# navganti/SIVO

Hardware: AMD Instinct MI355X
Metric: frames/sec, SIVO per-frame path (ORB+SegNet T=12+entropy) 352x1024 (higher is better)
Workload: dtype f32 (f16x3)

## Files before the change

### include/sivo_hip.h

```cpp
#ifndef SIVO_HIP_H
#define SIVO_HIP_H

#include <stddef.h>
#include <stdint.h>

#ifdef __cplusplus
extern "C" {
#endif

#define SIVO_OK 0
#define SIVO_ERR_INVALID_ARGUMENT 1
#define SIVO_ERR_RUNTIME 2
#define SIVO_ERR_UNSUPPORTED 3
#define SIVO_ERR_IMAGE_TOO_SMALL 4
#define SIVO_ERR_CAPACITY 5

const char *sivo_last_error(void);
int sivo_version(void);
int sivo_device_count(void);

typedef struct sivo_segnet *sivo_segnet_t;

int sivo_segnet_create(const char *prototxt_text, size_t prototxt_len, int t_override,
                       const float *weights, size_t n_weights, int device, sivo_segnet_t *out);
typedef struct SivoSegnetOptions {
    uint32_t struct_size;
    int32_t lanes;
    int32_t gemm;
    int32_t no_direct_f16x3;
    int32_t no_packed_activations;
    int32_t conv7_fp32;
    int32_t wino4_workspace_mb;
    int32_t debug_sync;
} SivoSegnetOptions;
int sivo_segnet_create_opts(const char *prototxt_text, size_t prototxt_len, int t_override, const float *weights, size_t n_weights,
                            int device, const SivoSegnetOptions *opts, sivo_segnet_t *out);
int sivo_caffemodel_weights(const char *prototxt_text, size_t prototxt_len, const void *model_bytes,
                            size_t model_len, float *out, size_t capacity, size_t *n_weights);
int sivo_segnet_create_from_files(const char *model_file, const char *weights_file, int t_override,
                                  int device, sivo_segnet_t *out);
int sivo_segnet_create_from_files_opts(const char *model_file, const char *weights_file, int t_override, int device,
                                       const SivoSegnetOptions *opts, sivo_segnet_t *out);
int sivo_segnet_create_multi(const char *prototxt_text, size_t prototxt_len, int t_override, const float *weights,
                             size_t n_weights, const int *device_ids, int ndev, sivo_segnet_t *out);
int sivo_segnet_create_multi_from_files(const char *model_file, const char *weights_file, int t_override,
                                        const int *device_ids, int ndev, sivo_segnet_t *out);
int sivo_segnet_create_multi_opts(const char *prototxt_text, size_t prototxt_len, int t_override, const float *weights, size_t n_weights,
                                  const int *device_ids, int ndev, const SivoSegnetOptions *opts, sivo_segnet_t *out);
int sivo_segnet_create_multi_from_files_opts(const char *model_file, const char *weights_file, int t_override, const int *device_ids,
                                             int ndev, const SivoSegnetOptions *opts, sivo_segnet_t *out);
int sivo_segnet_num_devices(sivo_segnet_t h, int *ndev);
int sivo_segnet_destroy(sivo_segnet_t h);
int sivo_segnet_shape(sivo_segnet_t h, int32_t *T, int32_t *C, int32_t *H, int32_t *W, int32_t *classes);
int sivo_segnet_num_params(const char *prototxt_text, size_t prototxt_len, size_t *n_params);

int sivo_segnet_forward_dev(sivo_segnet_t h, const uint8_t *d_bgr, int n_samples, int sample0,
// ... 22 lines not shown
int sivo_segnet_segment_logits_dev(sivo_segnet_t h, const uint8_t *d_bgr, uint64_t seed, uint8_t *d_classes,
                                   double *d_confidence, double *d_entropy, float *d_logits, void *stream);

int sivo_mc_segment_dev(const float *d_logits, int T, int classes, int64_t hw, uint8_t *d_classes,
                        double *d_confidence, double *d_entropy, void *stream);

int sivo_segnet_blob(sivo_segnet_t h, const char *name, float *host_out, size_t capacity, int32_t shape[4]);

int sivo_segnet_flops(sivo_segnet_t h, double *shared, double *per_sample);

typedef struct {
    char layer[64];
    char kernel[96];
    int32_t samples;
    int32_t launches;
    double flops_per_sample;
    double bytes_per_sample;
    double ms_total;
    int32_t kernel_launches;
    int32_t pad_;
} SivoOpProfile;
int sivo_segnet_profile(sivo_segnet_t h, int enable);
int sivo_segnet_profile_read(sivo_segnet_t h, SivoOpProfile *out, int capacity, int *n_out);

typedef struct SivoH3Layer {
    char layer[48];
    float vmax, vscale, uscale;
} SivoH3Layer;
int sivo_segnet_gemm_status(sivo_segnet_t h, int *mode, int *overflow_frames, SivoH3Layer *per_layer, int capacity, int *n_layers);
typedef struct SivoGuardLayer {
    char layer[48];
    char kernel[24];
    float rel_err, rel_rms, ref_max, first_rel_err;
    int32_t level;
} SivoGuardLayer;
int sivo_segnet_guard_report(sivo_segnet_t h, SivoGuardLayer *rows, int capacity, int *n_rows, float *budget, float *predicted,
                             float *logit_max, double *guard_ms, int *builds);
int sivo_segnet_take_overflow(sivo_segnet_t h, int *overflowed);

typedef struct {
    float x, y, size, angle, response;
    int32_t octave, class_id;
} SivoKeyPoint;

typedef struct sivo_orb *sivo_orb_t;

// ... 322 lines not shown
```

### sivo_amd/_lib.py

```python
import ctypes as C
import os
import threading

_HERE = os.path.dirname(os.path.abspath(__file__))
LIB_PATH = os.path.join(_HERE, "libsivo_hip.so")

OK = 0
ERR_INVALID_ARGUMENT = 1
ERR_RUNTIME = 2
ERR_UNSUPPORTED = 3
ERR_IMAGE_TOO_SMALL = 4
ERR_CAPACITY = 5


class SivoError(RuntimeError):
    def __init__(self, code, msg):
        super().__init__(f"libsivo_hip error {code}: {msg}")
        self.code = code


class SivoInvalidArgument(SivoError, ValueError):
    """SIVO_ERR_INVALID_ARGUMENT: where the reference throws std::invalid_argument."""


class KeyPoint(C.Structure):
    _fields_ = [("x", C.c_float), ("y", C.c_float), ("size", C.c_float), ("angle", C.c_float),
                ("response", C.c_float), ("octave", C.c_int32), ("class_id", C.c_int32)]


class OpProfile(C.Structure):
    _fields_ = [("layer", C.c_char * 64), ("kernel", C.c_char * 96), ("samples", C.c_int32), ("launches", C.c_int32),
                ("flops_per_sample", C.c_double), ("bytes_per_sample", C.c_double), ("ms_total", C.c_double),
                ("kernel_launches", C.c_int32), ("pad_", C.c_int32)]


class SegnetOptions(C.Structure):
    _fields_ = [("struct_size", C.c_uint32), ("lanes", C.c_int32), ("gemm", C.c_int32), ("no_direct_f16x3", C.c_int32),
                ("no_packed_activations", C.c_int32), ("conv7_fp32", C.c_int32), ("wino4_workspace_mb", C.c_int32), ("debug_sync", C.c_int32)]


class SearchQuery(C.Structure):
    _fields_ = [("u", C.c_float), ("v", C.c_float), ("radius", C.c_float), ("lvl_lo", C.c_int32), ("lvl_hi", C.c_int32),
                ("ur", C.c_float), ("gate", C.c_float), ("angle", C.c_float), ("flags", C.c_int32)]


class SearchRule(C.Structure):
    _fields_ = [("th_dist", C.c_int32), ("accept_lt", C.c_int32), ("ratio_mode", C.c_int32), ("nn_ratio", C.c_float),
                ("gate_mode", C.c_int32), ("check_orientation", C.c_int32), ("dynamic", C.c_int32), ("tie_last", C.c_int32),
                ("F12", C.c_float * 9), ("ex", C.c_float), ("ey", C.c_float)]


class Edge(C.Structure):
    _fields_ = [("pose", C.c_int32), ("point", C.c_int32), ("stereo", C.c_int32), ("pad_", C.c_int32),
                ("obs", C.c_double * 3), ("inv_sigma2", C.c_double)]


class Sim3Match(C.Structure):
    _fields_ = [("obs1", C.c_double * 2), ("inv_sigma2_1", C.c_double), ("obs2", C.c_double * 2), ("inv_sigma2_2", C.c_double),
                ("x1c", C.c_double * 3), ("x2c", C.c_double * 3)]


# ... 60 lines not shown
    "sivo_segnet_create_from_files_opts": [C.c_char_p, C.c_char_p, _i, _i, _vp, C.POINTER(_vp)],
    "sivo_segnet_create_multi_opts": [C.c_char_p, _sz, _i, _vp, _sz, _pi32, _i, _vp, C.POINTER(_vp)],
    "sivo_segnet_create_multi_from_files_opts": [C.c_char_p, C.c_char_p, _i, _pi32, _i, _vp, C.POINTER(_vp)],
    "sivo_caffemodel_weights": [C.c_char_p, _sz, _vp, _sz, _vp, _sz, C.POINTER(_sz)],
    "sivo_segnet_create_from_files": [C.c_char_p, C.c_char_p, _i, _i, C.POINTER(_vp)],
    "sivo_segnet_create_multi": [C.c_char_p, _sz, _i, _vp, _sz, _pi32, _i, C.POINTER(_vp)],
    "sivo_segnet_create_multi_from_files": [C.c_char_p, C.c_char_p, _i, _pi32, _i, C.POINTER(_vp)],
    "sivo_segnet_num_devices": [_vp, _pi32],
    "sivo_segnet_destroy": [_vp],
    "sivo_segnet_shape": [_vp, _pi32, _pi32, _pi32, _pi32, _pi32],
    "sivo_segnet_num_params": [C.c_char_p, _sz, C.POINTER(_sz)],
    "sivo_segnet_forward_dev": [_vp, _vp, _i, _i, _u64, _vp, _vp, _vp, _vp],
    "sivo_mc_finalize_dev": [_vp, _i, _i64, _i, _vp, _vp, _vp, _vp],
    "sivo_mc_reduce_dev": [_vp, _i, _i, _i64, _vp, _vp, _i, _vp],
    "sivo_mc_variance_dev": [_vp, _i, _i, _i64, _vp, _vp, _vp],
    "sivo_segnet_segment": [_vp, _vp, _i, _i, _u64, _vp, _vp, _vp],
    "sivo_segnet_segment_dev": [_vp, _vp, _u64, _vp, _vp, _vp, _vp],
    "sivo_segnet_segment_logits_dev": [_vp, _vp, _u64, _vp, _vp, _vp, _vp, _vp],
    "sivo_mc_segment_dev": [_vp, _i, _i, _i64, _vp, _vp, _vp, _vp],
    "sivo_segnet_blob": [_vp, C.c_char_p, _vp, _sz, _pi32],
    "sivo_segnet_flops": [_vp, C.POINTER(_d), C.POINTER(_d)],
    "sivo_segnet_profile": [_vp, _i],
    "sivo_segnet_profile_read": [_vp, _vp, _i, _pi32],
    "sivo_segnet_gemm_status": [_vp, _pi32, _pi32, _vp, _i, _pi32],
    "sivo_segnet_prefix_bands": [_vp, _i, _vp, _vp, _vp],
    "sivo_segnet_prefix_band_dev": [_vp, _vp, _i, _i, _vp, _vp],
    "sivo_segnet_forward_banded_dev": [_vp, _vp, _i, _i, _i, C.c_uint64, _vp, _vp, _vp],
    "sivo_segnet_guard_report": [_vp, _vp, _i, _pi32, _vp, _vp, _vp, _vp, _pi32],
    "sivo_segnet_take_overflow": [_vp, _pi32],
    "sivo_orb_create": [_i, _f, _i, _i, _i, _i, C.POINTER(_vp)],
    "sivo_orb_destroy": [_vp],
    "sivo_orb_set_gaussian": [_vp, _i],
    "sivo_orb_set_launch_mode": [_vp, _i],
    "sivo_orb_tables": [_vp, _vp, _vp, _vp, _vp, _vp],
    "sivo_orb_extract": [_vp, _vp, _i, _i, _i, _vp, _vp, _i, _pi32],
    "sivo_orb_extract_dev": [_vp, _vp, _i, _i, _i, _vp, _vp, _i, _pi32, _vp],
    "sivo_orb_extract_pair_dev": [_vp, _vp, _vp, _vp, _i, _i, _i, _i, _vp, _vp, _i, _pi32, _vp, _vp, _i, _pi32, _vp],
    "sivo_orb_profile": [_vp, _i],
    "sivo_orb_profile_read": [_vp, C.POINTER(_d), _pi32, C.POINTER(_d)],
    "sivo_orb_level": [_vp, _i, _vp, _sz, _pi32, _pi32],
    "sivo_orb_candidates": [_vp, _i, _vp, _i, _pi32],
    "sivo_orb_distribute": [_vp, _i, _i, _i, _i, _i, _i, _vp, _i, _pi32],
    "sivo_hamming_matrix_dev": [_vp, _i, _vp, _i, _vp, _vp],
    "sivo_hamming_matrix": [_vp, _i, _vp, _i, _vp],
    "sivo_hamming_argmin2_dev": [_vp, _i, _vp, _vp, _vp, _vp, _vp, _vp, _vp, _vp],
    "sivo_hamming_argmin2": [_vp, _i, _vp, _i, _vp, _vp, _vp, _vp, _vp, _vp],
# ... 141 lines not shown
```

### sivo_amd/api/bayesian_segnet/bayesian_segnet.hpp

```cpp
#ifndef BAYESIAN_SEGNET_BAYESIAN_SEGNET_HPP
#define BAYESIAN_SEGNET_BAYESIAN_SEGNET_HPP

#ifdef SIVO_HAVE_EIGEN
#include <Eigen/Eigen>
#else
#include "../compat/eigen_min.hpp"
#endif
#ifdef SIVO_HAVE_OPENCV
#include <opencv2/core/core.hpp>
#else
#include "../compat/cv_min.hpp"
#endif

#include <cstdint>
#include <string>
#include <vector>

#include "../../../include/sivo_hip.h"

struct sivo_segnet;

namespace SIVO {

#ifdef SIVO_HAVE_EIGEN
// ... 1 lines not shown
using MatXu = Eigen::Matrix<uint8_t, Eigen::Dynamic, Eigen::Dynamic, Eigen::RowMajor>;
#else
using MatXd = sivo_compat::RowMatrix<double>;
using MatXu = sivo_compat::RowMatrix<uint8_t>;
#endif

double computeEntropy(const double probability);

enum Classes {
    ROAD, SIDEWALK, BUILDING, WALL, POLE, TRAFFIC_LIGHT, TRAFFIC_SIGN, VEGETATION, TERRAIN, SKY, PERSON, CAR,
    COMMERCIAL_VEHICLE, BIKE, VOID = 255
};

struct BayesianSegNetParams {
    BayesianSegNetParams(const std::string model_filepath, const std::string weights_filepath)
        : model_file(model_filepath), weights_file(weights_filepath) {}
    bool use_gpu = true;
    std::string model_file;
    std::string weights_file;
    int monte_carlo_samples = 0;
    uint64_t seed = 0;
    int device = 0;
    std::vector<int> devices;
    SivoSegnetOptions options = {sizeof(SivoSegnetOptions), 0, 0, 0, 0, 0, 0, 0};
};

class BayesianSegNet {
 public:
    explicit BayesianSegNet(const BayesianSegNetParams &params);
    ~BayesianSegNet();
    BayesianSegNet(const BayesianSegNet &) = delete;
    BayesianSegNet &operator=(const BayesianSegNet &) = delete;

    void segmentImage(const cv::Mat &image, MatXu &classes, MatXd &confidence, MatXd &entropy);
    cv::Mat generateConfidenceImage(const MatXd &confidence);
    cv::Mat generateVarianceImage(MatXd &variance);
    cv::Mat generateEntropyImage(MatXd &entropy);
    cv::Mat generateSegmentedImage(const MatXu &classes, const cv::Mat &test_image);
    cv::Size getInputGeometry() { return this->input_geometry; }

 private:
    void checkConfig();
    void generateSegmentationColours();
    cv::Mat resizeImage(const cv::Mat &image);

    sivo_segnet *handle = nullptr;
    cv::Size input_geometry;
// ... 8 lines not shown
```

### sivo_amd/csrc/conv_wino4_h3.hip

```cpp
#include <hip/hip_runtime.h>
#include <stdint.h>

#include <cmath>
#include <cstdlib>
#include <cstring>
#include <vector>

#include "common.hpp"
#include "lds_dma.hpp"
#include "segnet_kernels.hpp"

namespace sivo {

typedef _Float16 half8 __attribute__((ext_vector_type(8)));
typedef float f32x16 __attribute__((ext_vector_type(16)));
typedef uint32_t u32x4 __attribute__((ext_vector_type(4)));
typedef int i32x4 __attribute__((ext_vector_type(4)));

constexpr int H3_KC = 32;

struct H3Args {
    const uint32_t *V;
    const unsigned char *U;
    float *M;
// ... 569 lines not shown
    for (int xi = 0; xi < 36; ++xi)
        for (int cb = 0; cb < ncb; ++cb)
            for (int s = 0; s < nst; ++s) {
                uint16_t *img = out.data() + ((size_t)(xi * ncb + cb) * nst + s) * 2048;
                for (int o = 0; o < 4; ++o)
                    for (int r = 0; r < 32; ++r)
                        for (int el = 0; el < 8; ++el) {
                            const float x = U[((size_t)xi * cin + s * H3_KC + 8 * o + el) * Kp + cb * 32 + r];
                            const uint32_t p = wino4_h3_pack_value(x, scale);
                            const size_t at = (size_t)(o * 32 + r) * 8 + el;
                            img[at] = (uint16_t)(p & 0xffffu);
                            img[1024 + at] = (uint16_t)(p >> 16);
                        }
            }
    return scale;
}

struct H3Tile { int bm, bn; };
static H3Tile h3_tile(int64_t P, int Kp) {
    if (Kp % 256) return {256, 128};
    const int64_t items_big = 36 * ((P + 255) / 256) * (Kp / 256);
    return {items_big >= 3 * 256 ? 256 : 128, 256};
}

void launch_wino4_gemm_h3(const uint32_t *V, const void *U, float *M, int C, int Kp, int P, int Pp, hipStream_t s) {
    static const bool lds_all = !(SIVO_DIAG_ENV("SIVO_H3_LDS_ALL") && std::atoi(SIVO_DIAG_ENV("SIVO_H3_LDS_ALL")) == 0);
    static const int force_tile = SIVO_DIAG_ENV("SIVO_H3_TILE") ? std::atoi(SIVO_DIAG_ENV("SIVO_H3_TILE")) : -1;
    static int attr_set[64] = {0};
    if (FirstUse once(attr_set); once) {
        for (const void *f : {(const void *)wino4_gemm_h3_kernel<256, 256>, (const void *)wino4_gemm_h3_kernel<128, 256>, (const void *)wino4_gemm_h3_kernel<256, 128>})
            SIVO_HIP(hipFuncSetAttribute(f, hipFuncAttributeMaxDynamicSharedMemorySize, 160 * 1024));
    }
    static const int n_cu = [] { hipDeviceProp_t pr; int d = 0; (void)hipGetDevice(&d); return hipGetDeviceProperties(&pr, d) == hipSuccess ? pr.multiProcessorCount : 256; }();
    const dim3 grid((unsigned)((n_cu / 8) * 8 > 0 ? (n_cu / 8) * 8 : 8));
    H3Args a{};
    a.V = V; a.U = static_cast<const unsigned char *>(U); a.M = M; a.C = C; a.Kp = Kp; a.P = P; a.Pp = Pp;
    H3Tile t = h3_tile(P, Kp);
    if (t.bn == 256 && (force_tile == 0 || force_tile == 1)) t.bm = force_tile == 0 ? 256 : 128;
    a.ptiles = (int)((P + t.bm - 1) / t.bm); a.ktiles = Kp / t.bn;
    const size_t lds = lds_all ? (size_t)160 * 1024 : (size_t)(2 * t.bm + 3 * t.bn) * 128;
#ifdef SIVO_DIAG
    if (const char *ab = SIVO_DIAG_ENV("SIVO_H3_ABL")) {
        a.ptiles = (P + 255) / 256; a.ktiles = Kp / 256;
#define H3_ABL_CASE(n)                                                                                                              \
    case n:                                                                                                                         \
        SIVO_HIP(hipFuncSetAttribute(reinterpret_cast<const void *>(wino4_gemm_h3_kernel<256, 256, n>), hipFuncAttributeMaxDynamicSharedMemorySize, 160 * 1024)); \
// ... 47 lines not shown
```

### sivo_amd/csrc/segnet.cpp

```cpp
#include "segnet_impl.hpp"

namespace sivo {

void harvest(sivo_segnet &S) {
    if (!S.pending) return;
    for (Op &op : S.ops) {
        if (!op.timed_mask) continue;
        int n = 0;
        for (int l = 0; l < Op::PROF_LANES; ++l) {
            if (!(op.timed_mask & (1u << l))) continue;
            float ms = 0.f;
            if (!op.w4_gemm_only_last) {
                SIVO_HIP(hipEventSynchronize(op.ev1[l]));
                SIVO_HIP(hipEventElapsedTime(&ms, op.ev0[l], op.ev1[l]));
                op.ms_total += ms;
            }
            for (int g = 0; g < op.w4_groups_last[l]; ++g)
                for (int k = op.w4_gemm_only_last ? 1 : 0; k < (op.w4_gemm_only_last ? 2 : 3); ++k) {
                    SIVO_HIP(hipEventSynchronize(op.w4_ev[l][4 * g + k + 1]));
                    SIVO_HIP(hipEventElapsedTime(&ms, op.w4_ev[l][4 * g + k], op.w4_ev[l][4 * g + k + 1]));
                    op.w4_ms[k] += ms;
                }
            op.w4_launches += op.w4_groups_last[l];
            op.w4_groups_last[l] = 0;
            op.kernel_launches += 1;
            n += op.lane_n[l];
        }
        op.last_n = n;
        op.launches += 1;
        op.timed_mask = 0;
    }
    S.pending = false;
// ... 166 lines not shown
        if (debug_sync) SIVO_HIP(hipDeviceSynchronize());
    }
}

void forward(sivo_segnet &S, const uint8_t *d_bgr, int n, int sample0, uint64_t seed, float *d_prob_sum,
             float *d_logits, float *d_prob, hipStream_t st, const McTargets *mc, const BandInput *pre) {
    const int64_t hw = (int64_t)S.H * S.W;
    S.last_seed = seed; S.last_sample0 = sample0;
    if (S.profile) harvest(S);
    h3_absorb(S);
    struct Pause {
        sivo_segnet &S; bool was;
        explicit Pause(sivo_segnet &s) : S(s), was(s.h3_on) { if (S.h3_pause) S.h3_on = false; S.h3_pause = false; }
        ~Pause() { S.h3_on = was; }
    } pause(S);
    const Blob &lg = S.blobs[S.logits_blob];
    if (lg.shared) throw std::runtime_error("the network has no test-time dropout: nothing to sample");
    if (!pre) launch_preprocess(d_bgr, (float *)S.blobs[S.input_blob].d, hw, st);
    const bool fuse = S.cls_op >= 0 && !d_prob && !d_logits && (mc || d_prob_sum || S.d_sum64);
    const size_t last = fuse ? (size_t)S.cls_op : S.ops.size();
    S.cls_pk_now = fuse && S.ops[S.cls_op].c3 && S.ops[S.cls_op].pk_in && S.ops[S.cls_op].d3_vscale > 0.f && S.pk_on && S.h3_on && !S.calibrating;
    size_t fork = 0;
    while (fork < last && (S.ops[fork].skip || S.blobs[S.ops[fork].out].shared)) ++fork;
    int lanes = S.d_wino4_ws ? S.ws_lanes : 2;
    if (S.profile && !S.profile_keep_lanes) lanes = 1;
    while (lanes > 1 && n < 2 * lanes) --lanes;
    while (lanes > 1 && fork < last && !S.ops[fork].skip && S.ops[fork].out2 >= 0 && S.blobs[S.ops[fork].out2].shared &&
           !S.blobs[S.ops[fork].out].shared)
        ++fork;
    if (pre) bands_unpack(S, *pre, n, sample0, seed, st, &fork);
    else run_ops(S, 0, fork, 0, n, sample0, seed, st, 0);
    if (lanes == 1) {
        run_ops(S, fork, last, 0, n, sample0, seed, st, 0);
    } else {
        if (!S.lane_fork) SIVO_HIP(hipEventCreateWithFlags(&S.lane_fork, hipEventDisableTiming));
        SIVO_HIP(hipEventRecord(S.lane_fork, st));
        int n0 = 0;
        for (int l = 0; l < lanes; ++l) {
            const int nl = n / lanes + (l < n % lanes ? 1 : 0);
            hipStream_t ls = st;
            if (l > 0) {
                if (!S.lane_stream[l]) {
                    SIVO_HIP(hipStreamCreateWithFlags(&S.lane_stream[l], hipStreamNonBlocking));
                    SIVO_HIP(hipEventCreateWithFlags(&S.lane_join[l], hipEventDisableTiming));
                }
                ls = S.lane_stream[l];
                SIVO_HIP(hipStreamWaitEvent(ls, S.lane_fork, 0));
            }
            run_ops(S, fork, last, n0, nl, sample0, seed, ls, l);
            if (l > 0) SIVO_HIP(hipEventRecord(S.lane_join[l], ls));
            n0 += nl;
        }
        for (int l = 1; l < lanes; ++l) SIVO_HIP(hipStreamWaitEvent(st, S.lane_join[l], 0));
    }
    if (fuse) {
        Op &op = S.ops[S.cls_op];
        const Blob &bi = S.blobs[op.in];
        ClsMcArgs a{};
        a.in = (const float *)bi.d; a.in_sample_stride = bi.chw();
        a.wt = op.d_w_mc; a.ep_scale = op.d_scale; a.ep_shift = op.d_shift;
        a.T = n; a.Cin = op.cin; a.H = bi.H; a.W = bi.W; a.C = op.cout; a.relu = op.relu;
        a.logits = mc ? mc->logits : nullptr;
// ... 471 lines not shown
                    p.ms_total = op.w4_ms[k];
                    p.launches = op.launches;
                    p.kernel_launches = op.w4_launches;
                    (void)groups;
                }
                continue;
            }
            SivoOpProfile &p = out[r++];
            std::memset(&p, 0, sizeof p);
            std::snprintf(p.layer, sizeof p.layer, "%s", op.name.c_str());
            const bool d3_on = op.d3 && h->h3_on && op.d3_vscale > 0.f && op.drop_site < 0 && op.pool_op < 0;
            std::snprintf(p.kernel, sizeof p.kernel, "%s", op.mc_fused_last ? (op.cls_h3_last ? "conv_cls_h3_kernel" : "conv_wino_cls_mc_kernel") : d3_on ? "conv3_h3_kernel" : (op.c7h3 && !(h->h3_on && op.d3_vscale > 0.f)) ? "conv7_x6_kernel" : op.kernel.c_str());
            p.samples = op.last_n;
            p.flops_per_sample = op.flops;
            p.bytes_per_sample = op.bytes;
            p.ms_total = op.ms_total;
            p.launches = op.launches;
            p.kernel_launches = op.kernel_launches;
        }
        return SIVO_OK;
    });
}

extern "C" int sivo_segnet_take_overflow(sivo_segnet_t h, int *overflowed) {
    return guarded([&] {
        if (!h || !overflowed) throw std::invalid_argument("null argument");
        if (h->multi) throw std::invalid_argument("a multi-device handle has synchronous entry points only: they recompute such a frame themselves");
        const bool now = h3_tripped(*h);
        *overflowed = (now || h->h3_unreported) ? 1 : 0;
        h->h3_unreported = false;
        return SIVO_OK;
    });
}

extern "C" int sivo_segnet_guard_report(sivo_segnet_t h, SivoGuardLayer *rows, int capacity, int *n_rows, float *budget, float *predicted,
                                        float *logit_max, double *guard_ms, int *builds) {
    return guarded([&] {
        if (!h) throw std::invalid_argument("null handle");
        if (h->multi) throw std::invalid_argument("per-device state: query the handles of a multi-device handle one by one");
        if (n_rows) *n_rows = (int)h->guard_rows.size();
        if (budget) *budget = h->guard_budget;
        if (logit_max) *logit_max = h->guard_logit_max;
        if (predicted) *predicted = h->guard_predicted;
        if (guard_ms) *guard_ms = h->guard_ms;
        if (builds) *builds = h->guard_builds;
        if (rows)
// ... 53 lines not shown
```

### sivo_amd/csrc/segnet_impl.hpp

```cpp
#pragma once
#include <cmath>
#include <cstdlib>
#include <cstring>
#include <fstream>
#include <map>
#include <memory>
#include <sstream>
#include <stdexcept>
#include <string>
#include <vector>

#include "common.hpp"
#include "prototxt.hpp"
#include "segnet_kernels.hpp"
#include "segnet_multi.hpp"
#include <chrono>
#include <algorithm>


namespace sivo {
bool looks_like_caffemodel(const std::string &bytes);
std::vector<float> weights_from_caffemodel(const std::string &bytes, const ProtoNet &net);

struct Blob {
    std::string name;
    int C = 0, H = 0, W = 0;
    bool shared = true;
    bool is_mask = false;
    int src_W = 0;
    void *d = nullptr;
    bool fused_away = false;
    int drop_pending = -1;
    void *d_pk = nullptr;
    int pk_Hp = 0, pk_Wp = 0;
    bool pk_fresh = false;
    float pk_scale = 0.f;
    uint32_t *d_bits = nullptr;
    int bits_Hp = 0, bits_Wp = 0;
    int64_t pk_sample_bytes() const { return (int64_t)(C / 8) * 2 * pk_Hp * pk_Wp * 16; }
    int64_t bits_sample_dwords() const { return (int64_t)(C / 8) * bits_Hp * bits_Wp; }
// ... 35 lines not shown
    int wino4_group = 1;
    static constexpr int PROF_LANES = 4;
    std::vector<hipEvent_t> w4_ev[PROF_LANES];
    double w4_ms[3] = {0.0, 0.0, 0.0};
    int w4_groups_last[PROF_LANES] = {0, 0, 0, 0}, w4_launches = 0;
    unsigned timed_mask = 0;
    bool w4_gemm_only_last = false;
    bool skip = false;
    bool w4_bridge = false;
    bool w4_bridged_in = false;
    int pool_op = -1;
    int unpool_in = -1, unpool_mask = -1;
    int drop_site = -1;
    bool drop_moved = false;
    int in_drop_site = -1;
    int guard_level = 0;
    int local_size = 5;
    float alpha = 0.f, beta = 0.f;
    double flops = 0.0;
    std::string name, kernel;
    hipEvent_t ev0[PROF_LANES] = {nullptr, nullptr, nullptr, nullptr}, ev1[PROF_LANES] = {nullptr, nullptr, nullptr, nullptr};
    double ms_total = 0.0, bytes = 0.0;
    int launches = 0, kernel_launches = 0, last_n = 0, lane_n[PROF_LANES] = {0, 0, 0, 0};
};


struct PrefixBands;
void free_bands(PrefixBands *);
}

struct sivo_segnet {
    SivoSegnetOptions opt{};
    sivo::SegnetMulti *multi = nullptr;
    sivo::ProtoNet proto;
    std::vector<float> prefix_weights;
    std::map<std::string, int> guard_levels_used;
    std::map<int, sivo::PrefixBands *> bands;
    bool owns_flag = true;
    uint64_t last_seed = 0;
    int last_sample0 = 0;
    int device = 0;
    int T = 0, C = 3, H = 0, W = 0, classes = 0;
    std::vector<sivo::Blob> blobs;
    std::vector<sivo::Op> ops;
    std::map<std::string, int> blob_id;
    int input_blob = -1, logits_blob = -1;
    int cls_op = -1;
    bool has_softmax = false;
    uint8_t *d_image = nullptr;
    float *d_prob_sum = nullptr;
    uint8_t *d_classes = nullptr;
    double *d_conf = nullptr, *d_ent = nullptr;
    hipStream_t stream = nullptr;
    int64_t sum_chunk = 0;
    double *d_sum64 = nullptr;
    double flops_shared = 0.0, flops_sample = 0.0;
    bool profile = false, pending = false;
    bool profile_mfma_only = false;
    bool profile_keep_lanes = false;
    std::vector<void *> owned;
    static constexpr int MAX_LANES = 4;
    int ws_lanes = 1;
    hipStream_t lane_stream[MAX_LANES] = {nullptr, nullptr, nullptr, nullptr};
    hipEvent_t lane_fork = nullptr, lane_join[MAX_LANES] = {nullptr, nullptr, nullptr, nullptr};
    bool h3_on = false, calibrating = false;
    bool pk_on = true;
    bool cls_pk_now = false;
    volatile uint32_t *h3_flag = nullptr;
    uint32_t *d_h3_vmax = nullptr;
    int h3_overflow_frames = 0;
    int h3_back_offs = 0;
    bool h3_pause = false;
    bool guard_over_budget = false;
    bool h3_unreported = false;
    struct GuardRow { std::string layer, kernel; float rel_err = 0.f, rel_rms = 0.f, ref_max = 0.f, first_rel_err = 0.f; int level = 0; };
    std::vector<GuardRow> guard_rows;
    float guard_budget = 0.f, guard_logit_max = 0.f, guard_predicted = 0.f;
    double guard_ms = 0.0;
    int guard_builds = 0;
    float *d_wino4_ws = nullptr;
    size_t wino4_ws_floats = 0;
    size_t wino4_slot_floats = 0;
    ~sivo_segnet() {
        if (multi) sivo::segnet_multi_destroy(multi);
        for (auto &kv : bands) sivo::free_bands(kv.second);
// ... 2 lines not shown
                if (op.ev0[l]) (void)hipEventDestroy(op.ev0[l]);
                if (op.ev1[l]) (void)hipEventDestroy(op.ev1[l]);
                for (hipEvent_t e : op.w4_ev[l]) (void)hipEventDestroy(e);
            }
        }
        for (void *p : owned) (void)hipFree(p);
        if (h3_flag && owns_flag) (void)hipHostFree(const_cast<uint32_t *>(h3_flag));
        if (stream) (void)hipStreamDestroy(stream);
        for (int l = 0; l < MAX_LANES; ++l) {
            if (lane_stream[l]) (void)hipStreamDestroy(lane_stream[l]);
            if (lane_join[l]) (void)hipEventDestroy(lane_join[l]);
        }
        if (lane_fork) (void)hipEventDestroy(lane_fork);
    }
};

namespace sivo {

SivoSegnetOptions segnet_options(const SivoSegnetOptions *opts);
size_t count_params(const ProtoNet &net);
std::unique_ptr<sivo_segnet> build(const ProtoNet &net, int t_override, const float *weights, size_t n_weights, int device,
                                   const SivoSegnetOptions &opt, const std::map<std::string, int> &guard_levels = {}, int prefix_rows = 0);

bool h3_flag_take(sivo_segnet &S);
void h3_back_off(sivo_segnet &S);
bool h3_tripped(sivo_segnet &S);
void h3_absorb(sivo_segnet &S);
std::vector<uint8_t> calibration_frame(int H, int W, int variant = 0);
void calibrate_h3(sivo_segnet &S);
std::unique_ptr<sivo_segnet> build_guarded(const ProtoNet &net, int t_override, const float *weights, size_t n_weights, int device,
                                           const SivoSegnetOptions &opt);

struct McTargets {
    uint8_t *classes;
    double *conf, *ent;
    float *logits;
};
struct BandInput { const void *slots; int world; };
void harvest(sivo_segnet &S);
void run_ops(sivo_segnet &S, size_t first, size_t last, int n0, int n, int sample0, uint64_t seed, hipStream_t st, int lane);
void forward(sivo_segnet &S, const uint8_t *d_bgr, int n, int sample0, uint64_t seed, float *d_prob_sum, float *d_logits,
             float *d_prob, hipStream_t st, const McTargets *mc = nullptr, const BandInput *pre = nullptr);

struct PrefixBands {
    int world = 0, fork = -1, pools = 0, rows_max = 0;
    struct Item { int blob; int shift; int elt; int C, H, W; size_t off; };
// ... 14 lines not shown
```

### sivo_amd/csrc/segnet_kernels.hpp

```cpp
#pragma once
#include <hip/hip_runtime.h>
#include <stdint.h>

#include <vector>

namespace sivo {

struct ConvArgs {
    const float *in;
    int64_t in_sample_stride;
    const float *wt;
    const float *ep_scale;
    const float *ep_shift;
    float *out;
    int N, Cin, H, W, Cout, CoutPad;
    int tiles_x, tiles_y;
    int relu;
    int drop_site;
    int in_drop_site = -1;
    int sample0;
    uint64_t seed;
    const uint8_t *unpool_mask = nullptr;
    int64_t unpool_mask_stride = 0;
    float *pool_out = nullptr;
// ... 19 lines not shown
void launch_conv(const ConvArgs &a, int ks, hipStream_t s);
bool conv2_supported(int ks);
int conv2_slab_floats(int ks, int cout);
void conv2_pack_weights(const float *W, int ks, int cin, int cout, std::vector<float> &out, int *cout_pad);
void launch_conv2(const ConvArgs &a, int ks, hipStream_t s);
bool wino_supported(int ks, int cin, int cout, int H, int W);
void wino_pack_weights(const float *W, int cin, int cout, int cfg, std::vector<float> &out, int *cout_pad);
void launch_conv_wino(const ConvArgs &a, int cfg, hipStream_t s);
int wino_slab_floats(int cfg);
int wino_chunks(int cfg, int cin);
int wino_cout_tile(int cfg);

bool wino4_supported(int ks, int cin, int cout, int H, int W);
int wino4_cout_pad(int cout);
void wino4_pack_weights(const float *W, int cin, int cout, std::vector<float> &out, int *cout_pad);
int wino4_group(int N, int cin, int cout, int H, int W, size_t budget_bytes);
bool wino4_x6_supported(int cin, int cout_pad);
void wino4_x6_pack_weights(const std::vector<float> &U, int cin, int cout_pad, std::vector<uint16_t> &out);
size_t wino4_workspace_floats(int group, int cin, int cout, int H, int W);
bool wino4_h3_supported(int cin, int cout_pad);
float wino4_h3_pack_weights(const std::vector<float> &U, int cin, int cout_pad, std::vector<uint16_t> &out);
uint32_t wino4_h3_pack_value(float x, float scale);
void launch_wino4_gemm_h3(const uint32_t *V, const void *U, float *M, int C, int Kp, int P, int Pp, hipStream_t s);
bool conv3_h3_supported(int ks, int cin, int cout, int H, int W, bool unpool);
float conv3_h3_pack_weights(const float *W, int cin, int cout, std::vector<uint16_t> &out);
void launch_conv3_h3(const ConvArgs &a, hipStream_t s);
void launch_absmax(const float *x, int64_t n, uint32_t *out_bits, hipStream_t s);
void launch_absdiff_max(const float *a, const float *b, int64_t n, uint32_t *out_bits, double *out_sums, hipStream_t s);
size_t pk_bytes(int N, int C, int Hp, int Wp);
void launch_pk_pack(const float *in, int64_t in_sample_stride, void *out, int N, int C, int H, int W, int Hp, int Wp, float scale,
                    uint32_t *h3_flag, hipStream_t s);
void launch_pk_unpack(const void *in, float *out, int N, int C, int H, int W, int Hp, int Wp, float scale, hipStream_t s);
void launch_pool_bits(const uint8_t *codes, uint32_t *bits, int N, int C, int Hq, int Wq, int Hp, int Wp, hipStream_t s);
bool conv7_x6_supported(int ks, int cin, int cout, int H, int W);
void conv7_x6_pack_weights(const float *W, int cin, int cout, std::vector<uint16_t> &out);
void launch_conv7_x6(const ConvArgs &a, hipStream_t s);
bool conv7_h3_supported(int ks, int cin, int cout, int H, int W);
float conv7_h3_pack_weights(const float *W, int cin, int cout, std::vector<uint16_t> &out);
void launch_conv7_h3(const ConvArgs &a, hipStream_t s);
bool wino4f_supported(int ks, int cin, int cout, int H, int W);
int wino4f_slab_floats();
void wino4f_pack_weights(const float *W, int cin, int cout, std::vector<float> &out, int *cout_pad);
void launch_conv_wino4f(const ConvArgs &a, hipStream_t s);

struct ClsMcArgs {
    const float *in;
// ... 87 lines not shown
```

### sivo_amd/csrc/segnet_plan.cpp

```cpp
#include "segnet_impl.hpp"

namespace sivo {

SivoSegnetOptions segnet_options(const SivoSegnetOptions *opts) {
    SivoSegnetOptions o{};
    if (opts) std::memcpy(&o, opts, std::min<size_t>(sizeof o, opts->struct_size));
    o.struct_size = sizeof o;
    if (o.lanes < 1 || o.lanes > sivo_segnet::MAX_LANES) {
        if (o.lanes != 0) throw std::invalid_argument("SivoSegnetOptions.lanes must be 0 (default) or 1 .. 4");
        o.lanes = 2;
    }
    if (o.gemm < 0 || o.gemm > 2) throw std::invalid_argument("SivoSegnetOptions.gemm must be 0 (f16x3), 1 (bf16x6) or 2 (fp32)");
    if (o.wino4_workspace_mb < 0) throw std::invalid_argument("SivoSegnetOptions.wino4_workspace_mb is negative");
    if (o.wino4_workspace_mb == 0) o.wino4_workspace_mb = 16384;
    return o;
}

size_t count_params(const ProtoNet &net) {
    std::map<std::string, int> ch;
    ch[net.input] = net.shape[1];
    size_t n = 0;
    for (const ProtoLayer &L : net.layers) {
        const int cin = L.bottom.empty() ? net.shape[1] : ch[L.bottom[0]];
        if (L.type == "Convolution") {
            n += (size_t)L.num_output * cin * L.kernel_size * L.kernel_size + (size_t)L.num_output;
            ch[L.top[0]] = L.num_output;
        } else if (L.type == "BN") {
            n += 2 * (size_t)cin;
            ch[L.top[0]] = cin;
        } else {
            for (auto &t : L.top) ch[t] = cin;
        }
    }
    return n;
}

int new_blob(sivo_segnet &S, const std::string &name, int C, int H, int W, bool shared, bool is_mask = false) {
    Blob b;
// ... 454 lines not shown
```

### sivo_amd/segnet.py

```python
import ctypes as C

import numpy as np
import torch

from . import _lib
from ._lib import check, dbg, lib

CLASSES = ["ROAD", "SIDEWALK", "BUILDING", "WALL", "POLE", "TRAFFIC_LIGHT", "TRAFFIC_SIGN", "VEGETATION",
           "TERRAIN", "SKY", "PERSON", "CAR", "COMMERCIAL_VEHICLE", "BIKE"]
VOID = 255


class BayesianSegNetParams:

    def __init__(self, model_file="", weights_file="", use_gpu=True, **options):
        self.model_file, self.weights_file, self.use_gpu = model_file, weights_file, use_gpu
        self.options = dict(options)


_GEMM = {"f16x3": 0, "": 0, "x6": 1, "bf16x6": 1, "f32": 2, "fp32": 2}


def segnet_options(lanes=None, gemm=None, direct_f16x3=None, packed_activations=None, conv7=None, wino4_workspace_mb=None, debug_sync=None):
    import os
    env = os.environ.get
    o = _lib.SegnetOptions()
    o.struct_size = C.sizeof(_lib.SegnetOptions)
    o.lanes = int(lanes if lanes is not None else env("SIVO_LANES", "0"))
    g = gemm if gemm is not None else env("SIVO_GEMM", "")
    o.gemm = _GEMM[g] if isinstance(g, str) else int(g)
    o.no_direct_f16x3 = int(not direct_f16x3) if direct_f16x3 is not None else int(env("SIVO_D3", "1") == "0")
    o.no_packed_activations = int(not packed_activations) if packed_activations is not None else int(env("SIVO_D3_PK", "1") == "0")
    o.conv7_fp32 = int(conv7 in ("f32", "fp32")) if conv7 is not None else int(env("SIVO_CONV7", "") == "f32")
    o.wino4_workspace_mb = int(wino4_workspace_mb if wino4_workspace_mb is not None else env("SIVO_WINO4_MB", "0"))
    o.debug_sync = int(bool(debug_sync)) if debug_sync is not None else int(env("SIVO_DEBUG_SYNC") is not None)
    return o


def _stream():
    return C.c_void_p(torch.cuda.current_stream().cuda_stream)


class BayesianSegNet:

    def __init__(self, params=None, prototxt=None, weights=None, T=0, device=0, devices=None, **options):
        h = C.c_void_p()
        opt = segnet_options(**dict(getattr(params, "options", {}) or {}, **options))
        self.options = opt
        po = C.byref(opt)
        self._L = lib()
        self.devices = list(devices) if devices is not None else None
        if params is not None:
            if not params.model_file:
                raise ValueError("model_file (.prototxt file) is empty!")
            if not params.weights_file:
                raise ValueError("weights_file (.caffemodel file) is empty!")
            if not params.use_gpu:
                raise _lib.SivoError(_lib.ERR_UNSUPPORTED, "use_gpu=false: this library has no CPU path")
# ... 99 lines not shown
        img = np.ascontiguousarray(image_bgr, np.uint8)
        classes = np.empty((self.H, self.W), np.uint8)
        conf = np.empty((self.H, self.W), np.float64)
        ent = np.empty((self.H, self.W), np.float64)
        check(self._L.sivo_segnet_segment(self._h, img.ctypes.data_as(C.c_void_p), img.shape[0], img.shape[1],
                                        C.c_uint64(seed), classes.ctypes.data_as(C.c_void_p),
                                        conf.ctypes.data_as(C.c_void_p), ent.ctypes.data_as(C.c_void_p)))
        return classes, conf, ent

    def profile(self, enable=True, reset=False, mfma_only=False, keep_lanes=False):
        mode = ((5 if reset else 6) if keep_lanes else (3 if reset else 4)) if (enable and mfma_only) else 2 if (enable and reset) else int(bool(enable))
        check(self._L.sivo_segnet_profile(self._h, mode))

    def profile_read(self):
        n = C.c_int32(0)
        check(self._L.sivo_segnet_profile_read(self._h, None, 0, C.byref(n)))
        arr = (_lib.OpProfile * n.value)()
        check(self._L.sivo_segnet_profile_read(self._h, arr, n.value, C.byref(n)))
        return [dict(layer=a.layer.decode(), kernel=a.kernel.decode(), samples=a.samples, launches=a.launches,
                     flops_per_sample=a.flops_per_sample, bytes_per_sample=a.bytes_per_sample, ms_total=a.ms_total,
                     kernel_launches=a.kernel_launches)
                for a in arr]

    def take_overflow(self):
        ov = C.c_int32()
        check(self._L.sivo_segnet_take_overflow(self._h, C.byref(ov)))
        return bool(ov.value)

    def gemm_status(self):
        class _Row(C.Structure):
            _fields_ = [("layer", C.c_char * 48), ("vmax", C.c_float), ("vscale", C.c_float), ("uscale", C.c_float)]
        mode, ov, n = C.c_int32(), C.c_int32(), C.c_int32()
        check(self._L.sivo_segnet_gemm_status(self._h, C.byref(mode), C.byref(ov), None, 0, C.byref(n)))
        rows = (_Row * max(n.value, 1))()
        check(self._L.sivo_segnet_gemm_status(self._h, C.byref(mode), C.byref(ov), rows, n.value, C.byref(n)))
        return mode.value, ov.value, [(r.layer.decode(), r.vmax, r.vscale, r.uscale) for r in rows[:n.value]]

    def guard_report(self):
        class _Row(C.Structure):
            _fields_ = [("layer", C.c_char * 48), ("kernel", C.c_char * 24), ("rel_err", C.c_float), ("rel_rms", C.c_float),
                        ("ref_max", C.c_float), ("first_rel_err", C.c_float), ("level", C.c_int32)]
        n, builds = C.c_int32(), C.c_int32()
        budget, pred, lmax, ms = C.c_float(), C.c_float(), C.c_float(), C.c_double()
        check(self._L.sivo_segnet_guard_report(self._h, None, 0, C.byref(n), C.byref(budget), C.byref(pred), C.byref(lmax), C.byref(ms), C.byref(builds)))
        rows = (_Row * max(n.value, 1))()
        check(self._L.sivo_segnet_guard_report(self._h, rows, n.value, C.byref(n), None, None, None, None, None))
# ... 106 lines not shown
    cls = torch.empty((H, W), dtype=torch.uint8, device=dev)
    conf = torch.empty((H, W), dtype=torch.float64, device=dev)
    ent = torch.empty((H, W), dtype=torch.float64, device=dev)
    check(lib().sivo_mc_segment_dev(logits.data_ptr(), T, K, H * W, cls.data_ptr(), conf.data_ptr(), ent.data_ptr(), _stream()))
    return cls, conf, ent


def mc_finalize(prob_sum, t_total):
    K, H, W = prob_sum.shape
    dev = prob_sum.device
    cls = torch.empty((H, W), dtype=torch.uint8, device=dev)
    conf = torch.empty((H, W), dtype=torch.float64, device=dev)
    ent = torch.empty((H, W), dtype=torch.float64, device=dev)
    check(lib().sivo_mc_finalize_dev(prob_sum.data_ptr(), K, H * W, t_total, cls.data_ptr(), conf.data_ptr(),
                                     ent.data_ptr(), _stream()))
    return cls, conf, ent


def mc_variance(prob, classes):
    T, K, H, W = prob.shape
    var = torch.empty((H, W), dtype=torch.float64, device=prob.device)
    check(lib().sivo_mc_variance_dev(prob.data_ptr(), T, K, H * W, classes.data_ptr(), var.data_ptr(), _stream()))
    return var
```

Baseline: 143.5.

## Plan per-lane sample split to minimize padded Winograd GEMM tile work

The MC-dropout samples were split evenly across concurrent lane streams. The split is now chosen by searching all lane-size splits and scoring each by the padded f16x3 Winograd GEMM work it produces, using each layer's tile height. When costs tie, the most balanced split wins, and the chosen plan is cached per sample count. A user-forced split option and introspection APIs are also added. The cost model counts total padded work rather than the slowest lane, so it may pick uneven splits that weaken overlap between lanes.

```diff
diff --git a/include/sivo_hip.h b/include/sivo_hip.h
--- a/include/sivo_hip.h
+++ b/include/sivo_hip.h
@@ -32,6 +32,7 @@
     int32_t conv7_fp32;
     int32_t wino4_workspace_mb;
     int32_t debug_sync;
+    int32_t lane_split[4];
 } SivoSegnetOptions;
 int sivo_segnet_create_opts(const char *prototxt_text, size_t prototxt_len, int t_override, const float *weights, size_t n_weights,
                             int device, const SivoSegnetOptions *opts, sivo_segnet_t *out);
@@ -100,6 +101,15 @@
 } SivoOpProfile;
 int sivo_segnet_profile(sivo_segnet_t h, int enable);
 int sivo_segnet_profile_read(sivo_segnet_t h, SivoOpProfile *out, int capacity, int *n_out);
+int sivo_segnet_profile_lanes(sivo_segnet_t h, int32_t *lane_samples, int capacity_rows, int *n_rows);
+
+typedef struct SivoLaneLayer {
+    int64_t tiles;
+    int32_t cin, kp;
+} SivoLaneLayer;
+int sivo_segnet_plan_lanes(const SivoLaneLayer *layers, int n_layers, int n_samples, int lanes, int32_t sizes[4], int *n_lanes);
+int sivo_segnet_lane_cost(const SivoLaneLayer *layers, int n_layers, const int32_t *sizes, int n_lanes, double *cost, int *padded_launches);
+int sivo_segnet_lanes(sivo_segnet_t h, int n_samples, int32_t sizes[4], int *n_lanes, SivoLaneLayer *layers, int capacity, int *n_layers);
 
 typedef struct SivoH3Layer {
     char layer[48];
diff --git a/sivo_amd/_lib.py b/sivo_amd/_lib.py
--- a/sivo_amd/_lib.py
+++ b/sivo_amd/_lib.py
@@ -36,7 +36,12 @@
 
 class SegnetOptions(C.Structure):
     _fields_ = [("struct_size", C.c_uint32), ("lanes", C.c_int32), ("gemm", C.c_int32), ("no_direct_f16x3", C.c_int32),
-                ("no_packed_activations", C.c_int32), ("conv7_fp32", C.c_int32), ("wino4_workspace_mb", C.c_int32), ("debug_sync", C.c_int32)]
+                ("no_packed_activations", C.c_int32), ("conv7_fp32", C.c_int32), ("wino4_workspace_mb", C.c_int32), ("debug_sync", C.c_int32),
+                ("lane_split", C.c_int32 * 4)]
+
+
+class LaneLayer(C.Structure):
+    _fields_ = [("tiles", C.c_int64), ("cin", C.c_int32), ("kp", C.c_int32)]
 
 
 class SearchQuery(C.Structure):
@@ -143,6 +148,10 @@
     "sivo_segnet_flops": [_vp, C.POINTER(_d), C.POINTER(_d)],
     "sivo_segnet_profile": [_vp, _i],
     "sivo_segnet_profile_read": [_vp, _vp, _i, _pi32],
+    "sivo_segnet_profile_lanes": [_vp, _vp, _i, _pi32],
+    "sivo_segnet_plan_lanes": [_vp, _i, _i, _i, _pi32, _pi32],
+    "sivo_segnet_lane_cost": [_vp, _i, _pi32, _i, C.POINTER(_d), _pi32],
+    "sivo_segnet_lanes": [_vp, _i, _pi32, _pi32, _vp, _i, _pi32],
     "sivo_segnet_gemm_status": [_vp, _pi32, _pi32, _vp, _i, _pi32],
     "sivo_segnet_prefix_bands": [_vp, _i, _vp, _vp, _vp],
     "sivo_segnet_prefix_band_dev": [_vp, _vp, _i, _i, _vp, _vp],
diff --git a/sivo_amd/api/bayesian_segnet/bayesian_segnet.hpp b/sivo_amd/api/bayesian_segnet/bayesian_segnet.hpp
--- a/sivo_amd/api/bayesian_segnet/bayesian_segnet.hpp
+++ b/sivo_amd/api/bayesian_segnet/bayesian_segnet.hpp
@@ -47,7 +47,7 @@
     uint64_t seed = 0;
     int device = 0;
     std::vector<int> devices;
-    SivoSegnetOptions options = {sizeof(SivoSegnetOptions), 0, 0, 0, 0, 0, 0, 0};
+    SivoSegnetOptions options = {sizeof(SivoSegnetOptions), 0, 0, 0, 0, 0, 0, 0, {0, 0, 0, 0}};
 };
 
 class BayesianSegNet {
diff --git a/sivo_amd/csrc/conv_wino4_h3.hip b/sivo_amd/csrc/conv_wino4_h3.hip
--- a/sivo_amd/csrc/conv_wino4_h3.hip
+++ b/sivo_amd/csrc/conv_wino4_h3.hip
@@ -615,6 +615,7 @@
     const int64_t items_big = 36 * ((P + 255) / 256) * (Kp / 256);
     return {items_big >= 3 * 256 ? 256 : 128, 256};
 }
+int wino4_h3_tile_bm(int64_t P, int Kp) { return h3_tile(P, Kp).bm; }
 
 void launch_wino4_gemm_h3(const uint32_t *V, const void *U, float *M, int C, int Kp, int P, int Pp, hipStream_t s) {
     static const bool lds_all = !(SIVO_DIAG_ENV("SIVO_H3_LDS_ALL") && std::atoi(SIVO_DIAG_ENV("SIVO_H3_LDS_ALL")) == 0);
diff --git a/sivo_amd/csrc/segnet.cpp b/sivo_amd/csrc/segnet.cpp
--- a/sivo_amd/csrc/segnet.cpp
+++ b/sivo_amd/csrc/segnet.cpp
@@ -5,9 +5,13 @@
 void harvest(sivo_segnet &S) {
     if (!S.pending) return;
     for (Op &op : S.ops) {
-        if (!op.timed_mask) continue;
+        if (!op.timed_mask) {
+            for (int l = 0; l < Op::PROF_LANES; ++l) op.harvested_lane_n[l] = 0;
+            continue;
+        }
         int n = 0;
         for (int l = 0; l < Op::PROF_LANES; ++l) {
+            op.harvested_lane_n[l] = op.timed_mask & (1u << l) ? op.lane_n[l] : 0;
             if (!(op.timed_mask & (1u << l))) continue;
             float ms = 0.f;
             if (!op.w4_gemm_only_last) {
@@ -220,9 +224,8 @@
     S.cls_pk_now = fuse && S.ops[S.cls_op].c3 && S.ops[S.cls_op].pk_in && S.ops[S.cls_op].d3_vscale > 0.f && S.pk_on && S.h3_on && !S.calibrating;
     size_t fork = 0;
     while (fork < last && (S.ops[fork].skip || S.blobs[S.ops[fork].out].shared)) ++fork;
-    int lanes = S.d_wino4_ws ? S.ws_lanes : 2;
-    if (S.profile && !S.profile_keep_lanes) lanes = 1;
-    while (lanes > 1 && n < 2 * lanes) --lanes;
+    int lane_size[4];
+    int lanes = forward_lanes(S, n, lane_size);
     while (lanes > 1 && fork < last && !S.ops[fork].skip && S.ops[fork].out2 >= 0 && S.blobs[S.ops[fork].out2].shared &&
            !S.blobs[S.ops[fork].out].shared)
         ++fork;
@@ -235,7 +238,7 @@
         SIVO_HIP(hipEventRecord(S.lane_fork, st));
         int n0 = 0;
         for (int l = 0; l < lanes; ++l) {
-            const int nl = n / lanes + (l < n % lanes ? 1 : 0);
+            const int nl = lane_size[l];
             hipStream_t ls = st;
             if (l > 0) {
                 if (!S.lane_stream[l]) {
@@ -753,6 +756,68 @@
     });
 }
 
+extern "C" int sivo_segnet_profile_lanes(sivo_segnet_t h, int32_t *lane_samples, int capacity_rows, int *n_rows) {
+    return guarded([&] {
+        if (!h || !n_rows) throw std::invalid_argument("null argument");
+        if (h->multi) throw std::invalid_argument("per-device state: query the handles of a multi-device handle one by one");
+        DeviceGuard dg(h->device);
+        harvest(*h);
+        int rows = 0;
+        for (const Op &op : h->ops) rows += op.wino4 ? (op.w4_bridged_in ? 2 : 3) : 1;
+        *n_rows = rows;
+        if (!lane_samples) return SIVO_OK;
+        if (capacity_rows < rows) return fail(SIVO_ERR_CAPACITY, "%d rows, capacity %d", rows, capacity_rows);
+        int r = 0;
+        for (const Op &op : h->ops)
+            for (int k = op.wino4 ? (op.w4_bridged_in ? 2 : 3) : 1; k > 0; --k, ++r)
+                for (int l = 0; l < Op::PROF_LANES; ++l) lane_samples[4 * r + l] = op.harvested_lane_n[l];
+        return SIVO_OK;
+    });
+}
+
+extern "C" int sivo_segnet_plan_lanes(const SivoLaneLayer *layers, int n_layers, int n_samples, int lanes, int32_t sizes[4], int *n_lanes) {
+    return guarded([&] {
+        if ((!layers && n_layers) || n_layers < 0 || !sizes || !n_lanes) throw std::invalid_argument("null argument");
+        if (n_samples < 1 || lanes < 1 || lanes > sivo_segnet::MAX_LANES) throw std::invalid_argument("n_samples >= 1, lanes 1 .. 4");
+        int z[4];
+        *n_lanes = plan_lane_split(layers, n_layers, n_samples, lanes, z);
+        for (int l = 0; l < 4; ++l) sizes[l] = z[l];
+        return SIVO_OK;
+    });
+}
+
+extern "C" int sivo_segnet_lane_cost(const SivoLaneLayer *layers, int n_layers, const int32_t *sizes, int n_lanes, double *cost, int *padded_launches) {
+    return guarded([&] {
+        if ((!layers && n_layers) || n_layers < 0 || !sizes) throw std::invalid_argument("null argument");
+        if (n_lanes < 1 || n_lanes > sivo_segnet::MAX_LANES) throw std::invalid_argument("n_lanes 1 .. 4");
+        int z[4] = {0, 0, 0, 0}, padded = 0;
+        for (int l = 0; l < n_lanes; ++l) {
+            if (sizes[l] < 1) throw std::invalid_argument("lane sizes >= 1");
+            z[l] = sizes[l];
+        }
+        const double c = lane_split_cost(layers, n_layers, z, n_lanes, &padded);
+        if (cost) *cost = c;
+        if (padded_launches) *padded_launches = padded;
+        return SIVO_OK;
+    });
+}
+
+extern "C" int sivo_segnet_lanes(sivo_segnet_t h, int n_samples, int32_t sizes[4], int *n_lanes, SivoLaneLayer *layers, int capacity, int *n_layers) {
+    return guarded([&] {
+        if (!h || !sizes || !n_lanes) throw std::invalid_argument("null argument");
+        if (h->multi) throw std::invalid_argument("per-device state: query the handles of a multi-device handle one by one");
+        if (n_samples < 1 || n_samples > h->T) throw std::invalid_argument("n_samples must be in [1, T]");
+        int z[4];
+        *n_lanes = forward_lanes(*h, n_samples, z);
+        for (int l = 0; l < 4; ++l) sizes[l] = z[l];
+        const std::vector<SivoLaneLayer> v = lane_layers(*h);
+        if (n_layers) *n_layers = (int)v.size();
+        if (layers)
+            for (int i = 0; i < capacity && i < (int)v.size(); ++i) layers[i] = v[(size_t)i];
+        return SIVO_OK;
+    });
+}
+
 extern "C" int sivo_segnet_take_overflow(sivo_segnet_t h, int *overflowed) {
     return guarded([&] {
         if (!h || !overflowed) throw std::invalid_argument("null argument");
diff --git a/sivo_amd/csrc/segnet_impl.hpp b/sivo_amd/csrc/segnet_impl.hpp
--- a/sivo_amd/csrc/segnet_impl.hpp
+++ b/sivo_amd/csrc/segnet_impl.hpp
@@ -16,6 +16,8 @@
 #include "segnet_multi.hpp"
 #include <chrono>
 #include <algorithm>
+#include <array>
+#include <functional>
 
 
 namespace sivo {
@@ -97,6 +99,7 @@
     hipEvent_t ev0[PROF_LANES] = {nullptr, nullptr, nullptr, nullptr}, ev1[PROF_LANES] = {nullptr, nullptr, nullptr, nullptr};
     double ms_total = 0.0, bytes = 0.0;
     int launches = 0, kernel_launches = 0, last_n = 0, lane_n[PROF_LANES] = {0, 0, 0, 0};
+    int harvested_lane_n[PROF_LANES] = {0, 0, 0, 0};
 };
 
 
@@ -136,6 +139,7 @@
     std::vector<void *> owned;
     static constexpr int MAX_LANES = 4;
     int ws_lanes = 1;
+    std::map<int, std::array<int, 4>> lane_plan;
     hipStream_t lane_stream[MAX_LANES] = {nullptr, nullptr, nullptr, nullptr};
     hipEvent_t lane_fork = nullptr, lane_join[MAX_LANES] = {nullptr, nullptr, nullptr, nullptr};
     bool h3_on = false, calibrating = false;
@@ -184,6 +188,11 @@
 std::unique_ptr<sivo_segnet> build(const ProtoNet &net, int t_override, const float *weights, size_t n_weights, int device,
                                    const SivoSegnetOptions &opt, const std::map<std::string, int> &guard_levels = {}, int prefix_rows = 0);
 
+double lane_split_cost(const SivoLaneLayer *layers, int n_layers, const int *sizes, int n_lanes, int *padded_launches = nullptr);
+int plan_lane_split(const SivoLaneLayer *layers, int n_layers, int n, int lanes, int sizes[4]);
+std::vector<SivoLaneLayer> lane_layers(const sivo_segnet &S);
+int forward_lanes(sivo_segnet &S, int n, int sizes[4]);
+
 bool h3_flag_take(sivo_segnet &S);
 void h3_back_off(sivo_segnet &S);
 bool h3_tripped(sivo_segnet &S);
diff --git a/sivo_amd/csrc/segnet_kernels.hpp b/sivo_amd/csrc/segnet_kernels.hpp
--- a/sivo_amd/csrc/segnet_kernels.hpp
+++ b/sivo_amd/csrc/segnet_kernels.hpp
@@ -65,6 +65,7 @@
 float wino4_h3_pack_weights(const std::vector<float> &U, int cin, int cout_pad, std::vector<uint16_t> &out);
 uint32_t wino4_h3_pack_value(float x, float scale);
 void launch_wino4_gemm_h3(const uint32_t *V, const void *U, float *M, int C, int Kp, int P, int Pp, hipStream_t s);
+int wino4_h3_tile_bm(int64_t P, int Kp);
 bool conv3_h3_supported(int ks, int cin, int cout, int H, int W, bool unpool);
 float conv3_h3_pack_weights(const float *W, int cin, int cout, std::vector<uint16_t> &out);
 void launch_conv3_h3(const ConvArgs &a, hipStream_t s);
diff --git a/sivo_amd/csrc/segnet_plan.cpp b/sivo_amd/csrc/segnet_plan.cpp
--- a/sivo_amd/csrc/segnet_plan.cpp
+++ b/sivo_amd/csrc/segnet_plan.cpp
@@ -10,10 +10,98 @@
         if (o.lanes != 0) throw std::invalid_argument("SivoSegnetOptions.lanes must be 0 (default) or 1 .. 4");
         o.lanes = 2;
     }
+    int forced = 0;
+    for (int l = 0; l < 4; ++l) {
+        if (o.lane_split[l] < 0 || (o.lane_split[l] > 0 && forced != l)) throw std::invalid_argument("SivoSegnetOptions.lane_split: sizes >= 1, lane 0 first, zeros behind them");
+        if (o.lane_split[l] > 0) ++forced;
+    }
+    if (forced) {
+        if (opts && opts->lanes != 0 && opts->lanes != forced) throw std::invalid_argument("SivoSegnetOptions.lanes differs from the number of lane_split sizes");
+        o.lanes = forced;
+    }
     if (o.gemm < 0 || o.gemm > 2) throw std::invalid_argument("SivoSegnetOptions.gemm must be 0 (f16x3), 1 (bf16x6) or 2 (fp32)");
     if (o.wino4_workspace_mb < 0) throw std::invalid_argument("SivoSegnetOptions.wino4_workspace_mb is negative");
     if (o.wino4_workspace_mb == 0) o.wino4_workspace_mb = 16384;
     return o;
+}
+
+double lane_split_cost(const SivoLaneLayer *layers, int n_layers, const int *sizes, int n_lanes, int *padded_launches) {
+    double products = 0.0;
+    int padded = 0;
+    for (int i = 0; i < n_layers; ++i)
+        for (int l = 0; l < n_lanes; ++l) {
+            const int64_t P = sizes[l] * layers[i].tiles;
+            const int bm = wino4_h3_tile_bm(P, layers[i].kp);
+            const int64_t groups = (P + bm - 1) / bm;
+            products += (double)(groups * bm) * layers[i].cin * layers[i].kp;
+            padded += P % bm != 0;
+        }
+    if (padded_launches) *padded_launches = padded;
+    return products;
+}
+
+int plan_lane_split(const SivoLaneLayer *layers, int n_layers, int n, int lanes, int sizes[4]) {
+    lanes = std::max(1, std::min(lanes, (int)sivo_segnet::MAX_LANES));
+    while (lanes > 1 && n < 2 * lanes) --lanes;
+    for (int l = 0; l < 4; ++l) sizes[l] = 0;
+    if (lanes == 1) { sizes[0] = n; return 1; }
+    int cur[4] = {0, 0, 0, 0};
+    double best = 0.0;
+    long best_spread = -1;
+    const auto spread = [&](const int *z) { long q = 0; for (int l = 0; l < lanes; ++l) q += (long)z[l] * z[l]; return q; };
+    const std::function<void(int, int, int)> walk = [&](int l, int left, int cap) {
+        if (l == lanes - 1) {
+            if (left < 2 || left > cap) return;
+            cur[l] = left;
+            const double c = lane_split_cost(layers, n_layers, cur, lanes);
+            const long q = spread(cur);
+            const bool tie = best_spread >= 0 && std::fabs(c - best) <= 1e-9 * std::max(c, best);
+            if (best_spread < 0 || (tie ? q < best_spread : c < best)) {
+                best = tie ? std::min(c, best) : c; best_spread = q;
+                for (int k = 0; k < lanes; ++k) sizes[k] = cur[k];
+            }
+            return;
+        }
+        for (int z = std::min(cap, left - 2 * (lanes - 1 - l)); z >= 2; --z) {
+            cur[l] = z;
+            walk(l + 1, left - z, z);
+        }
+    };
+    walk(0, n, n);
+    return lanes;
+}
+
+std::vector<SivoLaneLayer> lane_layers(const sivo_segnet &S) {
+    std::vector<SivoLaneLayer> v;
+    for (const Op &op : S.ops) {
+        if (op.kind != OP_CONV || op.skip || !op.wino4 || !op.d_wh3 || S.blobs[op.out].shared) continue;
+        const Blob &bi = S.blobs[op.in];
+        v.push_back(SivoLaneLayer{(int64_t)((bi.H + 3) / 4) * (bi.W / 4), op.cin, op.cout_pad});
+    }
+    return v;
+}
+
+int forward_lanes(sivo_segnet &S, int n, int sizes[4]) {
+    int lanes = S.d_wino4_ws ? S.ws_lanes : 2;
+    if (S.profile && !S.profile_keep_lanes) lanes = 1;
+    for (int l = 0; l < 4; ++l) sizes[l] = 0;
+    int forced = 0, sum = 0;
+    while (forced < 4 && S.opt.lane_split[forced] > 0) sum += S.opt.lane_split[forced++];
+    if (lanes > 1 && forced == lanes && sum == n) {
+        for (int l = 0; l < forced; ++l) sizes[l] = S.opt.lane_split[l];
+        return forced;
+    }
+    const int key = n * 8 + lanes;
+    auto it = S.lane_plan.find(key);
+    if (it == S.lane_plan.end()) {
+        const std::vector<SivoLaneLayer> layers = lane_layers(S);
+        std::array<int, 4> z{};
+        plan_lane_split(layers.data(), (int)layers.size(), n, lanes, z.data());
+        it = S.lane_plan.emplace(key, z).first;
+    }
+    int used = 0;
+    for (int l = 0; l < 4; ++l) { sizes[l] = it->second[(size_t)l]; used += sizes[l] > 0; }
+    return used;
 }
 
 size_t count_params(const ProtoNet &net) {
diff --git a/sivo_amd/segnet.py b/sivo_amd/segnet.py
--- a/sivo_amd/segnet.py
+++ b/sivo_amd/segnet.py
@@ -21,7 +21,8 @@
 _GEMM = {"f16x3": 0, "": 0, "x6": 1, "bf16x6": 1, "f32": 2, "fp32": 2}
 
 
-def segnet_options(lanes=None, gemm=None, direct_f16x3=None, packed_activations=None, conv7=None, wino4_workspace_mb=None, debug_sync=None):
+def segnet_options(lanes=None, gemm=None, direct_f16x3=None, packed_activations=None, conv7=None, wino4_workspace_mb=None, debug_sync=None,
+                   lane_split=None):
     import os
     env = os.environ.get
     o = _lib.SegnetOptions()
@@ -34,6 +35,13 @@
     o.conv7_fp32 = int(conv7 in ("f32", "fp32")) if conv7 is not None else int(env("SIVO_CONV7", "") == "f32")
     o.wino4_workspace_mb = int(wino4_workspace_mb if wino4_workspace_mb is not None else env("SIVO_WINO4_MB", "0"))
     o.debug_sync = int(bool(debug_sync)) if debug_sync is not None else int(env("SIVO_DEBUG_SYNC") is not None)
+    split = lane_split if lane_split is not None else [int(x) for x in env("SIVO_LANE_SPLIT", "").replace("+", ",").split(",") if x.strip()]
+    if len(split) > 4:
+        raise ValueError("lane_split: at most 4 lanes")
+    for l, z in enumerate(split):
+        o.lane_split[l] = int(z)
+    if not any(split):
+        o.struct_size = _lib.SegnetOptions.lane_split.offset
     return o
 
 
@@ -179,6 +187,21 @@
                      kernel_launches=a.kernel_launches)
                 for a in arr]
 
+    def profile_lanes(self):
+        n = C.c_int32(0)
+        check(self._L.sivo_segnet_profile_lanes(self._h, None, 0, C.byref(n)))
+        arr = (C.c_int32 * (4 * n.value))()
+        check(self._L.sivo_segnet_profile_lanes(self._h, arr, n.value, C.byref(n)))
+        return [tuple(arr[4 * r:4 * r + 4]) for r in range(n.value)]
+
+    def lanes(self, n_samples=None):
+        n = self.T if n_samples is None else n_samples
+        sizes, used, nl = (C.c_int32 * 4)(), C.c_int32(), C.c_int32()
+        check(self._L.sivo_segnet_lanes(self._h, n, sizes, C.byref(used), None, 0, C.byref(nl)))
+        rows = (_lib.LaneLayer * max(nl.value, 1))()
+        check(self._L.sivo_segnet_lanes(self._h, n, sizes, C.byref(used), rows, nl.value, C.byref(nl)))
+        return list(sizes[:used.value]), [(r.tiles, r.cin, r.kp) for r in rows[:nl.value]]
+
     def take_overflow(self):
         ov = C.c_int32()
         check(self._L.sivo_segnet_take_overflow(self._h, C.byref(ov)))
@@ -331,3 +354,18 @@
     var = torch.empty((H, W), dtype=torch.float64, device=prob.device)
     check(lib().sivo_mc_variance_dev(prob.data_ptr(), T, K, H * W, classes.data_ptr(), var.data_ptr(), _stream()))
     return var
+
+
+def plan_lanes(layers, n_samples, lanes=2):
+    rows = (_lib.LaneLayer * max(len(layers), 1))(*[_lib.LaneLayer(*map(int, r)) for r in layers])
+    sizes, used = (C.c_int32 * 4)(), C.c_int32()
+    check(lib().sivo_segnet_plan_lanes(rows, len(layers), n_samples, lanes, sizes, C.byref(used)))
+    return list(sizes[:used.value])
+
+
+def lane_cost(layers, sizes):
+    rows = (_lib.LaneLayer * max(len(layers), 1))(*[_lib.LaneLayer(*map(int, r)) for r in layers])
+    z = (C.c_int32 * len(sizes))(*sizes)
+    cost, padded = C.c_double(), C.c_int32()
+    check(lib().sivo_segnet_lane_cost(rows, len(layers), z, len(sizes), C.byref(cost), C.byref(padded)))
+    return cost.value, padded.value
```

Result: faster. 145.5, median of 6 (+1.4%).
